# PACTHEMAN123/spMV-test

Hardware: AMD Instinct MI355X
Metric: fp32 CSR SpMV: achieved HBM GB/s (rocprofv3 FETCH_SIZE + WRITE_SIZE bytes of the K steps / wall time) (higher is better)
Workload: dtype f32; 1 GPU; c4: 16777216 x 16777216, nnz 268435456, row lengths 'mixed' mean 16, banded columns (band 8192), seed 20251031; variant=auto, rows_per_gpu=16777216, nnz_per_gpu=268435456, parallelism=single GPU, devices=1 ranks on 1 device(s), launch=one process, algorithmic_bytes_per_gpu=2348810244, hbm_bytes_per_gpu=1840380781

## Files before the change

include/spmv_hip.h:

```cpp
#ifndef SPMV_HIP_H
#define SPMV_HIP_H

#include <stdint.h>

#if defined(__GNUC__)
#define SPMV_API __attribute__((visibility("default")))
#else
#define SPMV_API
#endif

#ifdef __cplusplus
extern "C" {
#endif

typedef struct spmv_csr spmv_csr_t;

enum spmv_status {
    SPMV_OK = 0,
    SPMV_ERR_NO_DEVICE = -1,
    SPMV_ERR_INVALID = -2,
    SPMV_ERR_HIP = -3,
    SPMV_ERR_VARIANT = -4,
    SPMV_ERR_NOT_PLANNED = -5,
    SPMV_ERR_STALE_PLAN = -6
// ... 96 lines not shown
SPMV_API int spmv_csr_color(const spmv_csr_t *a, uint32_t seed, void *stream, int32_t *d_color ,
                            int32_t *d_perm , int32_t *color_ptr , int cap ,
                            int64_t info[8]);
SPMV_API int spmv_csr_permute(const spmv_csr_t *a, const int32_t *d_row_perm ,
                              const int32_t *d_col_perm , int flags, void *stream, spmv_csr_t **out);
SPMV_API int spmv_csr_permute_values(spmv_csr_t *b, const spmv_csr_t *a, void *stream);
SPMV_API int spmv_csr_permute_gather(const spmv_csr_t *b, int count, const void *d_src, int64_t src_stride, void *d_dst,
                                     int64_t dst_stride, void *stream);
SPMV_API int64_t spmv_csr_permute_map_bytes(const spmv_csr_t *b);
SPMV_API int spmv_permute_vector(const int32_t *d_perm, int64_t n, int inverse, const float *d_src, float *d_dst, void *stream);

SPMV_API int spmv_csr_plan(spmv_csr_t *h, int variant, void *stream);
SPMV_API int spmv_csr_run(spmv_csr_t *h, int variant, const float *d_x, float *d_y, void *stream);

SPMV_API int spmv_csr_values_changed(spmv_csr_t *h);

SPMV_API int spmv_csr_plan_get(const spmv_csr_t *h, int variant, int32_t params[8]);
SPMV_API int spmv_csr_plan_set(spmv_csr_t *h, int variant, const int32_t params[8], void *stream);
SPMV_API int spmv_csr_plan_like(spmv_csr_t *dst, const spmv_csr_t *src, int variant, void *stream);

SPMV_API int64_t spmv_csr_plan_bytes(const spmv_csr_t *h, int variant);

SPMV_API int spmv_csr_plan_describe(const spmv_csr_t *h, int variant, char *buf, int n);

SPMV_API int spmv_csr_time(spmv_csr_t *h, int variant, const float *d_x, float *d_y, int iters,
                  void *stream, float *ms_per_launch);

SPMV_API int spmv_csr_run_host(spmv_csr_t *h, int variant, const float *x_host, float *y_host,
                               float *kernel_ms);

SPMV_API int spmv_csr_spmm_plan(spmv_csr_t *h, void *stream);
SPMV_API int spmv_csr_spmm(spmv_csr_t *h, int k, const float *d_X, int64_t ldx, float *d_Y, int64_t ldy, void *stream);
SPMV_API int64_t spmv_csr_spmm_plan_bytes(const spmv_csr_t *h);
SPMV_API int spmv_csr_spmm_describe(const spmv_csr_t *h, char *buf, int n);

SPMV_API int spmv_csr_sddmm(spmv_csr_t *h, int k, const float *d_U, int64_t ldu, const float *d_X, int64_t ldx,
                            float *d_out, void *stream);

SPMV_API int spmv_csr_row_softmax(spmv_csr_t *h, float scale, const float *d_scores, float *d_out, void *stream);
SPMV_API int spmv_csr_row_softmax_backward(spmv_csr_t *h, float scale, const float *d_P, const float *d_dP,
                                           float *d_dS, void *stream);

SPMV_API int spmv_csr_attention_plan(spmv_csr_t *h, void *stream);
SPMV_API int64_t spmv_csr_attention_plan_bytes(const spmv_csr_t *h);
SPMV_API int spmv_csr_attention_forward(spmv_csr_t *h, float scale, int k, const float *d_Q, int64_t ldq, const float *d_K,
                                        int64_t ldk, int kv, const float *d_V, int64_t ldv, float *d_O, int64_t ldo,
// ... 162 lines not shown
```

spmv-test_amd/capi.py:

```python
from __future__ import annotations

import ctypes as C
import os
from pathlib import Path

PKG_DIR = Path(__file__).resolve().parent
LIB_PATH = PKG_DIR / "lib" / "libspmv_hip.so"
LAUNCHERS_PATH = PKG_DIR / "lib" / "libspmv_launchers.so"
TESTER_PATH = PKG_DIR / "bin" / "sparse_sgemv"
DIST_LIB_PATH = PKG_DIR / "lib" / "libspmv_dist.so"
DIST_SELFTEST_PATH = PKG_DIR / "bin" / "spmv_dist_selftest"

SCALAR, WAVE, WAVE_PIPE, VECTOR, ADAPTIVE, TILED, PANEL, AUTO, XSKIP = range(9)
VARIANTS = {"scalar": SCALAR, "wave": WAVE, "wave_pipe": WAVE_PIPE, "vector": VECTOR,
            "adaptive": ADAPTIVE, "tiled": TILED, "panel": PANEL, "auto": AUTO}
ALL_VARIANTS = dict(VARIANTS, xskip=XSKIP)

OK, ERR_NO_DEVICE, ERR_INVALID, ERR_HIP, ERR_VARIANT, ERR_NOT_PLANNED, ERR_STALE_PLAN = 0, -1, -2, -3, -4, -5, -6

_i32p, _f32p, _vp = C.c_void_p, C.c_void_p, C.c_void_p
_H = C.c_void_p
_HP = C.POINTER(C.c_void_p)


# ... 59 lines not shown
    "spmv_csr_spmm_plan": (C.c_int, [_H, _vp]),
    "spmv_csr_spmm": (C.c_int, [_H, C.c_int, _f32p, C.c_int64, _f32p, C.c_int64, _vp]),
    "spmv_csr_spmm_plan_bytes": (C.c_int64, [_H]),
    "spmv_csr_spmm_describe": (C.c_int, [_H, C.c_char_p, C.c_int]),
    "spmv_csr_sddmm": (C.c_int, [_H, C.c_int, _f32p, C.c_int64, _f32p, C.c_int64, _f32p, _vp]),
    "spmv_csr_spmm_16": (C.c_int, [_H, C.c_int, C.c_int, _vp, C.c_int64, _vp, C.c_int64, _vp]),
    "spmv_csr_sddmm_16": (C.c_int, [_H, C.c_int, C.c_int, _vp, C.c_int64, _vp, C.c_int64, _f32p, _vp]),
    "spmv_csr_spmm_plan_cols": (C.c_int, [_H, C.c_int, _vp]),
    "spmv_csr_spmm_cols": (C.c_int, [_H, C.c_int, C.c_int, _vp, C.c_int64, _vp, C.c_int64, _vp]),
    "spmv_csr_sddmm_cols": (C.c_int, [_H, C.c_int, C.c_int, _vp, C.c_int64, _vp, C.c_int64, _f32p, _vp]),
    "spmv_csr_row_softmax": (C.c_int, [_H, C.c_float, _f32p, _f32p, _vp]),
    "spmv_csr_row_softmax_backward": (C.c_int, [_H, C.c_float, _f32p, _f32p, _f32p, _vp]),
    "spmv_csr_attention_plan": (C.c_int, [_H, _vp]),
    "spmv_csr_attention_plan_bytes": (C.c_int64, [_H]),
    "spmv_csr_attention_plan_heads": (C.c_int, [_H, C.c_int, _vp]),
    "spmv_csr_attention_max_heads": (C.c_int, [_H, C.c_int, C.c_int]),
    "spmv_csr_attention_plan_wide": (C.c_int, [_H, C.c_int, _vp]),
    "spmv_csr_attention_max_heads_wide": (C.c_int, [_H, C.c_int, C.c_int]),
    "spmv_csr_plan_get": (C.c_int, [_H, C.c_int, C.POINTER(C.c_int32)]),
    "spmv_csr_plan_set": (C.c_int, [_H, C.c_int, C.POINTER(C.c_int32), _vp]),
    "spmv_csr_plan_like": (C.c_int, [_H, _H, C.c_int, _vp]),
    "spmv_csr_plan_bytes": (C.c_int64, [_H, C.c_int]),
    "spmv_csr_plan_describe": (C.c_int, [_H, C.c_int, C.c_char_p, C.c_int]),
    "spmv_csr_time": (C.c_int, [_H, C.c_int, _f32p, _f32p, C.c_int, _vp, C.POINTER(C.c_float)]),
    "spmv_csr_run_host": (C.c_int, [_H, C.c_int, _f32p, _f32p, C.POINTER(C.c_float)]),
    "spmv_dense_gemv": (C.c_int, [C.c_int, C.c_int, _f32p, _f32p, _f32p, C.c_int, _vp]),
    "spmv_dense_gemv_workspace_bytes": (C.c_int64, [C.c_int, C.c_int]),
    "spmv_dense_gemv_ws": (C.c_int, [C.c_int, C.c_int, _f32p, _f32p, _f32p, C.c_int, _vp, C.c_int64, _vp]),
    "spmv_asp_retile": (C.c_int, [C.c_int, C.c_int, _f32p, _f32p, _vp]),
    "spmv_asp_gemv_ws": (C.c_int, [C.c_int, C.c_int, _f32p, _f32p, _f32p, _vp, C.c_int64, _vp]),
    "spmv_dense_gemv_host": (C.c_int, [C.c_int, C.c_int, _f32p, _f32p, _f32p, C.c_int, C.POINTER(C.c_float)]),
    "spmv_tcsr_from_dense_host": (C.c_int, [C.c_int, C.c_int, _f32p, _vp, _HP]),
    "spmv_tcsr_from_dense_device": (C.c_int, [C.c_int, C.c_int, _f32p, _vp, _HP]),
    "spmv_tcsr_sizes": (C.c_int, [_H, C.POINTER(C.c_int64), C.POINTER(C.c_int64), C.POINTER(C.c_int64)]),
    "spmv_tcsr_download": (C.c_int, [_H, _i32p, _i32p, _f32p]),
    "spmv_tcsr_run": (C.c_int, [_H, _f32p, _f32p, _vp]),
    "spmv_tcsr_run_host": (C.c_int, [_H, _f32p, _f32p, C.POINTER(C.c_float)]),
    "spmv_tcsr_destroy": (C.c_int, [_H]),
    "spmv_bitmap_from_dense_host": (C.c_int, [C.c_int, C.c_int, C.c_int, _f32p, _vp, _HP]),
    "spmv_bitmap_from_dense_device": (C.c_int, [C.c_int, C.c_int, C.c_int, _f32p, _vp, _HP]),
    "spmv_bitmap_sizes": (C.c_int, [_H, C.POINTER(C.c_int64), C.POINTER(C.c_int64), C.POINTER(C.c_int32)]),
    "spmv_bitmap_download": (C.c_int, [_H, _i32p, _f32p]),
    "spmv_bitmap_run": (C.c_int, [_H, _f32p, _f32p, _vp]),
    "spmv_bitmap_run_host": (C.c_int, [_H, _f32p, _f32p, C.POINTER(C.c_float)]),
    "spmv_bitmap_destroy": (C.c_int, [_H]),
    "spmv_synth_fill": (C.c_int, [C.c_uint64, C.c_int64, C.c_int64, C.c_int64, C.c_int64, C.c_int64,
# ... 768 lines not shown
        check(lib().spmv_csr_run_host(self._h, variant, _ptr(x), _ptr(y), C.byref(ms)))
        return ms.value

    def plan_params(self, variant: int):
        a = (C.c_int32 * 8)()
        check(lib().spmv_csr_plan_get(self._h, variant, a))
        return list(a)

    def plan_set(self, variant: int, params, stream=None) -> None:
        a = (C.c_int32 * 8)(*params)
        check(lib().spmv_csr_plan_set(self._h, variant, a, _stream_handle(stream)))

    def plan_like(self, other: "CsrMatrix", variant: int, stream=None) -> None:
        check(lib().spmv_csr_plan_like(self._h, other._h, variant, _stream_handle(stream)))

    def plan_describe(self, variant: int) -> str:
        buf = C.create_string_buffer(256)
        check(lib().spmv_csr_plan_describe(self._h, variant, buf, 256))
        return buf.value.decode()

    def plan_bytes(self, variant: int) -> int:
        return lib().spmv_csr_plan_bytes(self._h, variant)

    def download(self):
        import numpy as np
        rp = np.empty(self.rows + 1, np.int32)
        ci = np.empty(self.nnz, np.int32)
        va = np.empty(self.nnz, np.float32)
        check(lib().spmv_csr_download(self._h, _ptr(rp), _ptr(ci), _ptr(va)))
        return rp, ci, va

    def close(self) -> None:
        if self._h:
            check(lib().spmv_csr_destroy(self._h))
            self._h = C.c_void_p()
            self._keep = ()

    def __del__(self):
        try:
            self.close()
        except Exception:
            pass


class TcsrMatrix:

# ... 176 lines not shown
```

spmv-test_amd/csrc/capi.hip:

```cpp
#include <cctype>
#include <cstdarg>
#include <cstdint>
#include <cstdlib>
#include <cstring>
#include <new>
#include "spmv_internal.hpp"

namespace spmv {

static thread_local char g_err[512] = "";
static thread_local float g_first_launch_ms = 0.0f;

void set_error(const char *fmt, ...)
{
    va_list ap;
    va_start(ap, fmt);
    vsnprintf(g_err, sizeof g_err, fmt, ap);
    va_end(ap);
}

int hip_fail(hipError_t e, const char *what, const char *file, int line)
{
    set_error("HIP error %s:%d: %s (%s)", file, line, hipGetErrorString(e), what);
    return SPMV_ERR_HIP;
// ... 1825 lines not shown
        default: set_error("spmv_csr_plan_set: unknown variant %d", target); return SPMV_ERR_VARIANT;
    }
    if (rc == SPMV_OK && variant == SPMV_AUTO) h->auto_variant = target;
    return rc;
}

int spmv_csr_plan_like(spmv_csr_t *dst, const spmv_csr_t *src, int variant, void *stream)
{
    int32_t params[8];
    int rc = spmv_csr_plan_get(src, variant, params);
    return rc ? rc : spmv_csr_plan_set(dst, variant, params, stream);
}

int64_t spmv_csr_plan_bytes(const spmv_csr_t *h, int variant)
{
    if (!h) return 0;
    const PanelPlan &panel = variant == SPMV_AUTO ? h->plan_auto_panel : h->plan_panel;
    if (variant == SPMV_AUTO) variant = h->auto_variant;
    switch (variant) {
        case SPMV_ADAPTIVE:
            return (int64_t)(h->plan_adaptive.nchunks + 1) * 4 + (int64_t)h->plan_adaptive.nchunks * 8;
        case SPMV_TILED:
            return (int64_t)(h->plan_tiled.nchunks + 1) * 4 + (int64_t)h->plan_tiled.nchunks * 16 +
                   ((h->plan_tiled.n16 || h->plan_tiled.nsorted) ? (int64_t)h->plan_tiled.nchunks * 4 : 0) +
                   (int64_t)h->plan_tiled.n16 * 2 * h->plan_tiled.block * kNnzPerThread +
                   (int64_t)h->plan_tiled.nsorted * 4 * h->plan_tiled.block * kNnzPerThread +
                   (int64_t)h->plan_tiled.nblk_chunks * 256 * 4;
        case SPMV_XSKIP:
            return (int64_t)h->plan_xskip.nseg * 8 + ((int64_t)h->plan_xskip.nblocks + 1) * 4 +
                   (h->plan_xskip.slabs > 1 ? (int64_t)h->plan_xskip.nblocks * h->plan_xskip.slabs * 1024 * 8 : 0);
        case SPMV_PANEL: return panel_plan_bytes(panel, h->nnz);
        case SPMV_WAVE:
            if (h->nnz > 32 * h->rows) return 0;
            return (int64_t)h->plan_wave.n_long * 8 + (int64_t)h->plan_wave.pieces * 16;
        case SPMV_SCALAR:
        case SPMV_WAVE_PIPE:
            return (int64_t)h->plan_wave.n_long * 8 + (int64_t)h->plan_wave.pieces * 16 + h->plan_wave.blocks * 8;
        default: return 0;
    }
}

int spmv_csr_plan_describe(const spmv_csr_t *h, int variant, char *buf, int n)
{
    if (!h || !buf || n <= 0) { set_error("spmv_csr_plan_describe: bad argument"); return SPMV_ERR_INVALID; }
    const PanelPlan *panel = &h->plan_panel;
    if (variant == SPMV_AUTO) {
        if (h->auto_variant < 0) { snprintf(buf, (size_t)n, "not planned"); return SPMV_OK; }
        const int w = snprintf(buf, (size_t)n, "auto -> %s: ", spmv_variant_name(h->auto_variant));
        if (w < 0 || w >= n) return SPMV_OK;
        if (h->auto_variant != SPMV_PANEL) return spmv_csr_plan_describe(h, h->auto_variant, buf + w, n - w);
        panel = &h->plan_auto_panel;
        variant = SPMV_PANEL;
        buf += w;
        n -= w;
    }
    const ChunkPlan *p = variant == SPMV_ADAPTIVE ? &h->plan_adaptive : (variant == SPMV_TILED ? &h->plan_tiled : nullptr);
    if (variant == SPMV_VECTOR) snprintf(buf, (size_t)n, "lanes_per_row=%d", h->vector_width);
    else if (variant == SPMV_WAVE && h->nnz > 32 * h->rows) snprintf(buf, (size_t)n, "no plan (a wavefront per row)");
    else if (variant == SPMV_WAVE_PIPE || variant == SPMV_SCALAR || variant == SPMV_WAVE) {
        if (!h->plan_wave.ready) snprintf(buf, (size_t)n, "not planned (the first run plans)");
        else snprintf(buf, (size_t)n, "long_rows=%d pieces=%d block_rows=%d blocks=%lld blocks_with_x_window=%lld col16=%d", h->plan_wave.n_long,
                      h->plan_wave.pieces, h->plan_wave.block_rows, (long long)h->plan_wave.blocks, (long long)h->plan_wave.win_blocks,
// ... 286 lines not shown
```

spmv-test_amd/csrc/kernels_adaptive.hip:

```cpp
#include "spmv_internal.hpp"
#include "tiled_chunks.hpp"
#include "lane_group.hpp"

namespace spmv {

__device__ __forceinline__ int pad_idx(int i) { return i + (i >> 5); }
template <int BLOCK>
__device__ __forceinline__ void zero_pad_words(float *smem, int tid)
{
    for (int h = tid; h < (chunk_of(BLOCK) >> 5); h += BLOCK) smem[h * 33 + 32] = 0.0f;
}

__device__ __forceinline__ int xcd_chunk(int bid, int n)
{
    const int q = n / kXcds, rem = n % kXcds;
    const int j = bid % kXcds, idx = bid / kXcds;
    return j * q + (j < rem ? j : rem) + idx;
}

struct Segment {
    int s, e;
    float *dst;
};

// ... 433 lines not shown
}

template <int BLOCK, bool TILED, bool PERSIST, typename E = float>
__global__ __launch_bounds__(BLOCK, waves_per_simd(BLOCK, PERSIST))
void k_adaptive(int64_t rows, int64_t nnz, int64_t cols, int chunk0, int nrun, const int32_t *__restrict__ row_ptr,
                const int32_t *__restrict__ col_idx, const E *__restrict__ vals, const float *__restrict__ x,
                float *__restrict__ y, const int32_t *__restrict__ chunk_lb, float *__restrict__ carry,
                const int32_t *__restrict__ win, const int32_t *__restrict__ list, int kRegion)
{
    extern __shared__ __attribute__((aligned(16))) float smem[];
    __shared__ ChunkShared<BLOCK> sh;
    adaptive_body<BLOCK, TILED, PERSIST, E>(smem, sh, (int)blockIdx.x, (int)gridDim.x, rows, nnz, cols, chunk0, nrun, row_ptr,
                                            col_idx, vals, x, y, chunk_lb, carry, win, list, kRegion);
}


__device__ __forceinline__ unsigned col16_at(const u4 (&raw)[2], int j, int q)
{
    const int e = (j & 1) * 4 + q;
    const unsigned word = raw[j >> 1][e >> 1];
    return (e & 1) ? (word >> 16) : (word & 0xffffu);
}

template <int BLOCK, bool BLOCKS, typename E = float>
__device__ __forceinline__ void tiled16_body(float *smem, ChunkShared<BLOCK> &sh, int bid, int64_t rows, int64_t cols,
                                             int nrun, const int32_t *__restrict__ row_ptr,
                                             const uint16_t *__restrict__ col16, const E *__restrict__ vals,
                                             const float *__restrict__ x, float *__restrict__ y,
                                             const int32_t *__restrict__ chunk_lb, float *__restrict__ carry,
                                             const int32_t *__restrict__ win, const int32_t *__restrict__ list,
                                             int kRegionArg, const int32_t *__restrict__ blk)
{
    constexpr int kVec = kNnzPerThread / 4;
    static_assert(kNnzPerThread == 16, "the col16 lane layout is two 16-byte loads of eight offsets");

    const int tid = threadIdx.x;
    const int ci = xcd_chunk(bid, nrun);
    const ChunkHead h = chunk_head<BLOCK>(sh, tid, list ? list[ci] : ci, chunk_lb);
    const int c = h.c;
    const int w0 = win[2 * c];
    const int wl = win[2 * c + 1];
    const int wlen = wl & kLenMask;
    const bool by_blocks = BLOCKS && (wl & kBlockBit);
    const int kRegion = by_blocks ? (kRegionArg / kBlkCols) * kBlkCols : kRegionArg;

    u4 raw[2];
    vals4_t<E> vv[kVec];
    {
        const u4 *c8 = reinterpret_cast<const u4 *>(col16 + h.base);
        const vals4_t<E> *v4 = value_vectors(vals, h.base);
        raw[0] = __builtin_nontemporal_load(&c8[tid]);
        raw[1] = __builtin_nontemporal_load(&c8[BLOCK + tid]);
#pragma unroll
        for (int j = 0; j < kVec; ++j) vv[j] = stream_load<BLOCK>(v4, tid, j);
    }
    const RowBounds b0 = first_bounds(tid, h, row_ptr);

    f4 xv[kVec];
#pragma unroll
    for (int j = 0; j < kVec; ++j)
#pragma unroll
        for (int q = 0; q < 4; ++q) xv[j][q] = 0.0f;
    if (wlen <= kRegion && wlen > 0) {
        if (by_blocks) stage_blocks<BLOCK>(x, blk + (int64_t)c * kBlkMax, wlen / kBlkCols, cols, smem, tid);
        else stage_slice<BLOCK, true>(x, (int64_t)w0, wlen, cols, smem, tid);
        __syncthreads();
#pragma unroll
        for (int j = 0; j < kVec; ++j)
#pragma unroll
            for (int q = 0; q < 4; ++q) xv[j][q] = smem[col16_at(raw, j, q)];
        __syncthreads();
    } else {
        for (int off = 0; off < wlen; off += kRegion) {
            const int len = (wlen - off) < kRegion ? (wlen - off) : kRegion;
            const int64_t g0 = (int64_t)w0 + off;
            if (by_blocks) stage_blocks<BLOCK>(x, blk + (int64_t)c * kBlkMax + off / kBlkCols, len / kBlkCols, cols, smem, tid);
            else stage_slice<BLOCK, true>(x, g0, len, cols, smem, tid);
            __syncthreads();
#pragma unroll
            for (int j = 0; j < kVec; ++j)
#pragma unroll
                for (int q = 0; q < 4; ++q) {
                    const unsigned o = col16_at(raw, j, q) - (unsigned)off;
                    if (o < (unsigned)len) xv[j][q] = smem[o];
                }
            __syncthreads();
        }
    }

    stage_products<BLOCK, E>(smem, tid, vv, [&](int j, int q, int) { return xv[j][q]; });
    __syncthreads();
    reduce_chunk<BLOCK, true, BLOCKS ? 1 : 0>(smem, sh, tid, h.c, h.lb0, h.m, h.base, h.lim, row_ptr, y, carry, b0.rb, b0.re);
}

template <int BLOCK, bool BLOCKS, typename E = float>
__global__ __launch_bounds__(BLOCK, 8)
void k_tiled16(int64_t rows, int64_t cols, int nrun, const int32_t *__restrict__ row_ptr, const uint16_t *__restrict__ col16,
               const E *__restrict__ vals, const float *__restrict__ x, float *__restrict__ y,
               const int32_t *__restrict__ chunk_lb, float *__restrict__ carry, const int32_t *__restrict__ win,
               const int32_t *__restrict__ list, int kRegion, const int32_t *__restrict__ blk)
{
    extern __shared__ __attribute__((aligned(16))) float smem[];
    __shared__ ChunkShared<BLOCK> sh;
    tiled16_body<BLOCK, BLOCKS, E>(smem, sh, (int)blockIdx.x, rows, cols, nrun, row_ptr, col16, vals, x, y, chunk_lb, carry, win,
                                   list, kRegion, blk);
}

template <int BLOCK, typename E = float>
__device__ __forceinline__ void sorted_body(float *smem, ChunkShared<BLOCK> &sh, int bid, int64_t rows, int nrun,
                                            const int32_t *__restrict__ row_ptr, const uint32_t *__restrict__ perm,
                                            const E *__restrict__ vals, const float *__restrict__ x,
                                            float *__restrict__ y, const int32_t *__restrict__ chunk_lb,
                                            float *__restrict__ carry, const int32_t *__restrict__ win,
                                            const int32_t *__restrict__ list)
{
    constexpr int kChunkT = chunk_of(BLOCK);
    constexpr int kVec = kNnzPerThread / 4;
    constexpr int kColBits = sorted_col_bits(BLOCK);
    constexpr unsigned kColMask = (1u << kColBits) - 1u;

    const int tid = threadIdx.x;
    const int ci = xcd_chunk(bid, nrun);
    const ChunkHead h = chunk_head<BLOCK>(sh, tid, list[ci], chunk_lb);
    const float *xw = x + win[2 * h.c];

    u4 pw[kVec];
    vals4_t<E> vv[kVec];
    {
        const u4 *p4 = reinterpret_cast<const u4 *>(perm + (int64_t)ci * kChunkT);
        const vals4_t<E> *v4 = value_vectors(vals, h.base);
#pragma unroll
        for (int j = 0; j < kVec; ++j) pw[j] = stream_load<BLOCK>(p4, tid, j);
#pragma unroll
        for (int j = 0; j < kVec; ++j) vv[j] = stream_load<BLOCK>(v4, tid, j);
    }
    const RowBounds b0 = first_bounds(tid, h, row_ptr);

#pragma unroll
    for (int j = 0; j < kVec; ++j) {
        float g[4];
#pragma unroll
        for (int q = 0; q < 4; ++q) g[q] = xw[pw[j][q] & kColMask];
#pragma unroll
        for (int q = 0; q < 4; ++q) smem[pad_idx((int)(pw[j][q] >> kColBits))] = g[q];
    }
    __syncthreads();
    stage_products<BLOCK, E>(smem, tid, vv, [&](int, int, int w) { return smem[w]; });
    __syncthreads();
    reduce_chunk<BLOCK, true>(smem, sh, tid, h.c, h.lb0, h.m, h.base, h.lim, row_ptr, y, carry, b0.rb, b0.re);
}

template <int BLOCK, typename E = float>
__global__ __launch_bounds__(BLOCK, 8)
void k_sorted(int64_t rows, int nrun, const int32_t *__restrict__ row_ptr, const uint32_t *__restrict__ perm,
              const E *__restrict__ vals, const float *__restrict__ x, float *__restrict__ y,
              const int32_t *__restrict__ chunk_lb, float *__restrict__ carry, const int32_t *__restrict__ win,
              const int32_t *__restrict__ list)
{
    extern __shared__ __attribute__((aligned(16))) float smem[];
    __shared__ ChunkShared<BLOCK> sh;
    sorted_body<BLOCK, E>(smem, sh, (int)blockIdx.x, rows, nrun, row_ptr, perm, vals, x, y, chunk_lb, carry, win, list);
}

template <int BLOCK, bool BLOCKS, typename E = float>
__global__ __launch_bounds__(BLOCK, 8)
void k_tiled_mixed(int64_t rows, int64_t nnz, int64_t cols, int n32, int nsorted, int n16, const int32_t *__restrict__ row_ptr,
                   const int32_t *__restrict__ col_idx, const uint16_t *__restrict__ col16, const uint32_t *__restrict__ perm,
                   const E *__restrict__ vals, const float *__restrict__ x, float *__restrict__ y,
                   const int32_t *__restrict__ chunk_lb, float *__restrict__ carry, const int32_t *__restrict__ win,
                   const int32_t *__restrict__ list32, const int32_t *__restrict__ list_sorted,
                   const int32_t *__restrict__ list16, int kRegion, const int32_t *__restrict__ blk)
{
    extern __shared__ __attribute__((aligned(16))) float smem[];
    __shared__ ChunkShared<BLOCK> sh;
    const int b = (int)blockIdx.x;
    if (b < n32)
        adaptive_body<BLOCK, true, false, E>(smem, sh, b, n32, rows, nnz, cols, 0, n32, row_ptr, col_idx, vals, x,
                                             y, chunk_lb, carry, win, list32, kRegion);
    else if (b < n32 + nsorted)
        sorted_body<BLOCK, E>(smem, sh, b - n32, rows, nsorted, row_ptr, perm, vals, x, y, chunk_lb, carry, win, list_sorted);
    else
        tiled16_body<BLOCK, BLOCKS, E>(smem, sh, b - n32 - nsorted, rows, cols, n16, row_ptr, col16, vals, x, y, chunk_lb,
                                       carry, win, list16, kRegion, blk);
}

__global__ void k_carry_fixup(int nchunks, int chunk, const int32_t *__restrict__ row_ptr,
                              const int32_t *__restrict__ chunk_lb, const float *__restrict__ carry,
                              float *__restrict__ y)
{
    int c = blockIdx.x * blockDim.x + threadIdx.x;
    if (c >= nchunks - 1) return;
    const int lb0 = chunk_lb[c], lb1 = chunk_lb[c + 1];
    if (lb1 == lb0) return;
    const int64_t r = (int64_t)lb1 - 1;
    const int64_t endp = row_ptr[r + 1];
    if (endp <= (int64_t)(c + 1) * chunk) return;
    float s = y[r];
    for (int64_t c2 = c + 1; c2 * chunk < endp; ++c2) s += carry[c2];
    y[r] = s;
}

__global__ __launch_bounds__(256)
void k_plan_windows(int64_t nnz, int64_t cols, int nchunks, int chunk, const int32_t *__restrict__ col_idx,
                    int32_t *__restrict__ win, int32_t *__restrict__ stats, int region, int maxpass, int sorted_from,
                    int sorted_span, PlanCost cost, const int32_t *__restrict__ lb, const int32_t *__restrict__ row_ptr)
{
// ... 145 lines not shown
    int grid = nrun;
    if (PERSIST) {
        const int res = resident_workgroups(h.device, BLOCK, waves_per_simd(BLOCK, true));
        if (grid > res) grid = res;
    }
    return launch_region<k_adaptive<BLOCK, TILED, PERSIST, E>>("k_adaptive", h, p, grid, BLOCK, s, h.rows, h.nnz, h.cols, chunk0, nrun,
                                                               h.d_row_ptr, h.d_col_idx, vals, x, y, p.d_lb, p.d_carry, p.d_win,
                                                               (const int32_t *)nullptr, p.region);
}

template <int BLOCK, bool BLOCKS, typename E>
static int launch_tiled16(const spmv_csr &h, const ChunkPlan &p, const E *vals, const float *x, float *y, hipStream_t s)
{
    if (p.n16 <= 0) return SPMV_OK;
    return launch_region<k_tiled16<BLOCK, BLOCKS, E>>("k_tiled16", h, p, p.n16, BLOCK, s, h.rows, h.cols, p.n16, h.d_row_ptr, p.d_col16,
                                                      vals, x, y, p.d_lb, p.d_carry, p.d_win,
                                                      p.n16 == p.nchunks ? (const int32_t *)nullptr : p.d_list16.get(), p.region, p.d_blk);
}

template <int BLOCK, bool BLOCKS, typename E>
static int launch_mixed(const spmv_csr &h, const ChunkPlan &p, const E *vals, const float *x, float *y, hipStream_t s)
{
    const int n32 = p.nchunks - p.n16 - p.nsorted;
    return launch_region<k_tiled_mixed<BLOCK, BLOCKS, E>>("k_tiled_mixed", h, p, p.nchunks, BLOCK, s, h.rows, h.nnz, h.cols, n32, p.nsorted,
                                                          p.n16, h.d_row_ptr, h.d_col_idx, p.d_col16, p.d_perm, vals, x, y, p.d_lb,
                                                          p.d_carry, p.d_win, p.d_list32, p.d_list_sorted, p.d_list16, p.region, p.d_blk);
}

template <int BLOCK, typename E>
static int launch_sorted(const spmv_csr &h, const ChunkPlan &p, const E *vals, const float *x, float *y, hipStream_t s)
{
    return launch_region<k_sorted<BLOCK, E>>("k_sorted", h, p, p.nsorted, BLOCK, s, h.rows, p.nsorted, h.d_row_ptr, p.d_perm, vals, x,
                                             y, p.d_lb, p.d_carry, p.d_win, p.d_list_sorted);
}

template <int BLOCK, bool TILED, typename E>
static int launch_either(bool persist, const spmv_csr &h, const ChunkPlan &p, const E *vals, const float *x, float *y, hipStream_t s)
{
    if constexpr (TILED) {
        if (!persist && (p.n16 > 0 || p.nsorted > 0)) {
            const bool lists = p.nblk_chunks > 0;
            if (p.n16 == p.nchunks)
                return lists ? launch_tiled16<BLOCK, true>(h, p, vals, x, y, s) : launch_tiled16<BLOCK, false>(h, p, vals, x, y, s);
            if (p.nsorted == p.nchunks) return launch_sorted<BLOCK>(h, p, vals, x, y, s);
            return lists ? launch_mixed<BLOCK, true>(h, p, vals, x, y, s) : launch_mixed<BLOCK, false>(h, p, vals, x, y, s);
        }
    }
    if constexpr (kIs16<E>) {
        return launch_range<BLOCK, TILED, false>(h, p, vals, 0, p.nchunks, x, y, s);
// ... 49 lines not shown
```

spmv-test_amd/csrc/plan_adaptive.hip:

```cpp
#include <climits>
#include <cstdlib>
#include <cstring>
#include "spmv_internal.hpp"
#include "tiled_chunks.hpp"

namespace spmv {

__global__ void k_plan_chunks(int64_t rows, int nchunks, int chunk, const int32_t *__restrict__ row_ptr,
                              int32_t *__restrict__ lb)
{
    int c = blockIdx.x * blockDim.x + threadIdx.x;
    if (c > nchunks) return;
    if (c == nchunks) { lb[c] = (int32_t)rows; return; }
    const int64_t key = (int64_t)c * chunk;
    int64_t lo = 0, hi = rows;
    while (lo < hi) {
        int64_t mid = (lo + hi) >> 1;
        if ((int64_t)row_ptr[mid] < key) lo = mid + 1; else hi = mid;
    }
    lb[c] = (int32_t)lo;
}

template <int BLOCK>
__global__ __launch_bounds__(BLOCK) void k_plan_sorted(const int32_t *__restrict__ col_idx,
// ... 335 lines not shown
        p.nblk_chunks = 0;
        (void)p.d_col16.reset();
        (void)p.d_blk.reset();
    }
    return SPMV_OK;
}

static int count_block_list_chunks(const spmv_csr &h, ChunkPlan &p, hipStream_t s, int *out)
{
    *out = 0;
    if (p.nchunks == 0 || !p.d_win) return SPMV_OK;
    DevPtr<int32_t> nblk, some;
    SPMV_HIP_TRY(nblk.alloc(1));
    SPMV_HIP_TRY(some.alloc(1));
    SPMV_HIP_TRY(hipMemsetAsync(nblk.get(), 0, sizeof(int32_t), s));
    if (int rc = run_plan_col16(h, p, nullptr, nblk.get(), some.get(), 1, s)) return rc;
    int32_t cnt = 0;
    SPMV_HIP_TRY(hipMemcpyAsync(&cnt, nblk.get(), sizeof cnt, hipMemcpyDeviceToHost, s));
    SPMV_HIP_TRY(hipStreamSynchronize(s));
    *out = cnt;
    return SPMV_OK;
}

static int build_lists(const spmv_csr &h, ChunkPlan &p, hipStream_t s)
{
    (void)p.d_list16.reset();
    (void)p.d_list32.reset();
    (void)p.d_list_sorted.reset();
    (void)p.d_perm.reset();
    p.n16 = p.nsorted = 0;
    if (p.nchunks == 0 || !p.d_win || p.persist) return SPMV_OK;
    int rc;
    DevPtr<int32_t> f16, fs, t16, ts;
    SPMV_HIP_TRY(f16.alloc((size_t)p.nchunks));
    SPMV_HIP_TRY(fs.alloc((size_t)p.nchunks));
    SPMV_HIP_TRY(t16.alloc(1));
    SPMV_HIP_TRY(ts.alloc(1));
    const unsigned g = (unsigned)((p.nchunks + 255) / 256);
    hipLaunchKernelGGL(k_plan_kinds, dim3(g), dim3(256), 0, s, p.nchunks, p.d_win, f16.get(), fs.get());
    if ((rc = check_launch("k_plan_kinds"))) return rc;
    if ((rc = exclusive_scan_i32(f16.get(), p.nchunks, t16.get(), s))) return rc;
    if ((rc = exclusive_scan_i32(fs.get(), p.nchunks, ts.get(), s))) return rc;
    int32_t n16 = 0, ns = 0;
    SPMV_HIP_TRY(hipMemcpyAsync(&n16, t16.get(), sizeof(int32_t), hipMemcpyDeviceToHost, s));
    SPMV_HIP_TRY(hipMemcpyAsync(&ns, ts.get(), sizeof(int32_t), hipMemcpyDeviceToHost, s));
    SPMV_HIP_TRY(hipStreamSynchronize(s));
    p.n16 = n16;
    p.nsorted = ns;
    if (n16 == 0 && ns == 0) return SPMV_OK;
    SPMV_HIP_TRY(p.d_list16.alloc((size_t)n16));
    SPMV_HIP_TRY(p.d_list_sorted.alloc((size_t)ns));
    SPMV_HIP_TRY(p.d_list32.alloc((size_t)(p.nchunks - n16 - ns)));
    hipLaunchKernelGGL(k_plan_lists, dim3(g), dim3(256), 0, s, p.nchunks, p.d_win, f16.get(), fs.get(), p.d_list16, p.d_list_sorted,
                       p.d_list32);
    if ((rc = check_launch("k_plan_lists"))) return rc;
    if (ns > 0) {
        SPMV_HIP_TRY(p.d_perm.alloc((size_t)chunk_of(p.block) * (size_t)ns));
        rc = dispatch_block(p.block, [&](auto B) {
            constexpr int BLOCK = decltype(B)::value;
            hipLaunchKernelGGL((k_plan_sorted<BLOCK>), dim3(p.nchunks), dim3(BLOCK), 0, s, h.d_col_idx, p.d_win, fs.get(), p.d_perm);
            return check_launch("k_plan_sorted");
        });
        if (rc) return rc;
    }
    SPMV_HIP_TRY(hipStreamSynchronize(s));
    return SPMV_OK;
}

static int finish_tiled(spmv_csr &h, bool col16, hipStream_t s)
{
    int rc = col16 ? build_col16(h, h.plan_tiled, s) : SPMV_OK;
    if (rc == SPMV_OK) rc = build_lists(h, h.plan_tiled, s);
    if (rc) h.plan_tiled = ChunkPlan{};
    return rc;
}

int plan_tiled_with(spmv_csr &h, int block, int maxpass, bool col16, hipStream_t s)
{
    if ((block != 256 && block != 512 && block != 1024) || maxpass < 1 || maxpass > 64) {
        set_error("tiled plan: block %d / maxpass %d outside 256|512|1024 / 1..64", block, maxpass);
        return SPMV_ERR_INVALID;
    }
    const int rc = build_plan(h, block, maxpass, s, h.plan_tiled, nullptr, nullptr);
    return rc ? rc : finish_tiled(h, col16, s);
}

int plan_adaptive_with(spmv_csr &h, int block, hipStream_t s)
{
// ... 146 lines not shown
```

spmv-test_amd/csrc/spmv_internal.hpp:

```cpp
#pragma once
#include <hip/hip_runtime.h>
#include <atomic>
#include <cstdint>
#include <cstdio>
#include <utility>
#include "spmv_hip.h"
#include "attention_args.hpp"

namespace spmv {

void set_error(const char *fmt, ...) __attribute__((format(printf, 1, 2)));
int hip_fail(hipError_t e, const char *what, const char *file, int line);

#define SPMV_HIP_TRY(call)                                                   \
    do {                                                                     \
        hipError_t e__ = (call);                                             \
        if (e__ != hipSuccess) return ::spmv::hip_fail(e__, #call, __FILE__, __LINE__); \
    } while (0)

static inline int check_launch(const char *what)
{
    hipError_t e = hipGetLastError();
    if (e != hipSuccess) return hip_fail(e, what, __FILE__, __LINE__);
    return SPMV_OK;
// ... 46 lines not shown
constexpr int kMaxHeads = 65535;

#ifndef SPMV_T_NPT
#define SPMV_T_NPT 16
#endif
#ifndef SPMV_T_SHORT
#define SPMV_T_SHORT 32
#endif
constexpr int kNnzPerThread = SPMV_T_NPT;
constexpr int kShortSeg = SPMV_T_SHORT;

struct ChunkPlan {
    int block = 0;
    int nchunks = 0;
    DevPtr<int32_t> d_lb;
    DevPtr<float> d_carry;
    DevPtr<int32_t> d_win;
    DevPtr<uint16_t> d_col16;
    DevPtr<int32_t> d_list16;
    DevPtr<int32_t> d_list32;
    int n16 = 0;
    DevPtr<uint32_t> d_perm;
    DevPtr<int32_t> d_list_sorted;
    int nsorted = 0;
    int nsorted_marked = 0;
    int sorted_from = 0;
    int long_piece_chunks = 0;
    double model_cost = 0.0;
    DevPtr<int32_t> d_blk;
    int nblk_chunks = 0;
    int maxpass = 0;
    bool col16_wanted = false;
    int spanning_rows = 0;
    int region = 0;
    bool persist = false;
    int staged_single = 0;
    int staged_full = 0;
};

struct ValuesStamp {
    uint64_t gen = 0;
    uint64_t sum = 0;
    bool have_sum = false;
};

enum class PanelLayout { none = 0, sweep_l2 = 1, sweep_lds = 2, sorted_blocks = 3, binned = 4, binned_scattered = 5 };
// ... 435 lines not shown
```

spmv-test_amd/csrc/tiled_chunks.hpp:

```cpp
#pragma once
#include <type_traits>
#include "spmv_internal.hpp"

namespace spmv {

using i4 = int __attribute__((ext_vector_type(4)));
using f4 = float __attribute__((ext_vector_type(4)));
using u4 = unsigned __attribute__((ext_vector_type(4)));

#ifndef SPMV_T_GROUP
#define SPMV_T_GROUP 16
#endif
constexpr int kGroup = SPMV_T_GROUP;

__host__ __device__ constexpr int chunk_of(int block) { return block * kNnzPerThread; }
__host__ __device__ constexpr int prod_words(int block) { return chunk_of(block) + (chunk_of(block) >> 5); }
__host__ __device__ constexpr int region_words(int block) { return (block / 256) * 4832; }
static_assert(region_words(256) >= prod_words(256), "region must hold the products");
__host__ __device__ constexpr int max_long(int block) { return chunk_of(block) / (kShortSeg + 1) + 2; }
#ifndef SPMV_T_HUGE
#define SPMV_T_HUGE 512
#endif
constexpr int kHugeSeg = SPMV_T_HUGE;
__host__ __device__ constexpr int max_huge(int block) { return chunk_of(block) / (kHugeSeg + 1) + 2; }

template <typename F>
int dispatch_block(int block, F &&f)
{
    if (block == 256) return f(std::integral_constant<int, 256>{});
    if (block == 512) return f(std::integral_constant<int, 512>{});
    return f(std::integral_constant<int, 1024>{});
}

constexpr int kOutsideBit = 1 << 30;
constexpr int kCol16Bit = 1 << 29;
constexpr int kBlockBit = 1 << 28;
constexpr int kSortedBit = 1 << 27;
constexpr int kLenMask = kSortedBit - 1;
#ifndef SPMV_T_SORTED_FROM
#define SPMV_T_SORTED_FROM (-1)
#endif
constexpr int kSortedFromDefault = SPMV_T_SORTED_FROM;
__host__ __device__ constexpr int sorted_pos_bits(int block) { return block == 1024 ? 14 : (block == 512 ? 13 : 12); }
__host__ __device__ constexpr int sorted_col_bits(int) { return 18; }
static_assert(sorted_pos_bits(1024) + sorted_col_bits(1024) <= 32, "one word per nonzero");
#ifndef SPMV_T_BLKBITS
#define SPMV_T_BLKBITS 8
#endif
constexpr int kBlkBits = SPMV_T_BLKBITS;
constexpr int kBlkCols = 1 << kBlkBits;
constexpr int kBlkMax = 65536 / kBlkCols;

struct PlanCost {
    int c16_base = 788, c16_pass = 110, c32_base = 1075, c32_pass = 123, sorted_base = 1075, sorted_line_512 = 1792,
        sorted_line_1024 = 1485, sorted_few_rows = 205, unstaged = 3072, long_piece = 512;
};

int launch_plan_windows(const spmv_csr &h, const ChunkPlan &p, int32_t *d_stats, const PlanCost &cost, hipStream_t s);

}
```

Baseline: 5479 GB/s.

## Run mixed tiled chunks in identity order instead of per-format lists

When most chunks use the col16 format, the mixed tiled kernel maps each block straight to its chunk in natural order and branches on the window flags, instead of reading list16/list_sorted/list32 indirection arrays. Value vectors are loaded before dispatch so the stream load can be issued early. The last partial chunk is swapped so it is not scheduled last. The intent is to keep neighbouring chunks' x windows adjacent in time, which should improve reuse of x in L2, and to drop the list lookups. The cost is a divergent branch per block and a mix of chunk formats within each wave of blocks. An optional window-first staging switch is added but is off by default.

```diff
diff --git a/include/spmv_hip.h b/include/spmv_hip.h
--- a/include/spmv_hip.h
+++ b/include/spmv_hip.h
@@ -142,6 +142,8 @@
 SPMV_API int64_t spmv_csr_plan_bytes(const spmv_csr_t *h, int variant);
 
 SPMV_API int spmv_csr_plan_describe(const spmv_csr_t *h, int variant, char *buf, int n);
+
+SPMV_API int spmv_csr_plan_chunk_order(const spmv_csr_t *h, int variant);
 
 SPMV_API int spmv_csr_time(spmv_csr_t *h, int variant, const float *d_x, float *d_y, int iters,
                   void *stream, float *ms_per_launch);
diff --git a/spmv-test_amd/capi.py b/spmv-test_amd/capi.py
--- a/spmv-test_amd/capi.py
+++ b/spmv-test_amd/capi.py
@@ -105,6 +105,7 @@
     "spmv_csr_plan_like": (C.c_int, [_H, _H, C.c_int, _vp]),
     "spmv_csr_plan_bytes": (C.c_int64, [_H, C.c_int]),
     "spmv_csr_plan_describe": (C.c_int, [_H, C.c_int, C.c_char_p, C.c_int]),
+    "spmv_csr_plan_chunk_order": (C.c_int, [_H, C.c_int]),
     "spmv_csr_time": (C.c_int, [_H, C.c_int, _f32p, _f32p, C.c_int, _vp, C.POINTER(C.c_float)]),
     "spmv_csr_run_host": (C.c_int, [_H, C.c_int, _f32p, _f32p, C.POINTER(C.c_float)]),
     "spmv_dense_gemv": (C.c_int, [C.c_int, C.c_int, _f32p, _f32p, _f32p, C.c_int, _vp]),
@@ -919,6 +920,12 @@
     def plan_bytes(self, variant: int) -> int:
         return lib().spmv_csr_plan_bytes(self._h, variant)
 
+    def plan_chunk_order(self, variant: int) -> int:
+        rc = lib().spmv_csr_plan_chunk_order(self._h, variant)
+        if rc < 0:
+            check(rc)
+        return rc
+
     def download(self):
         import numpy as np
         rp = np.empty(self.rows + 1, np.int32)
diff --git a/spmv-test_amd/csrc/capi.hip b/spmv-test_amd/csrc/capi.hip
--- a/spmv-test_amd/csrc/capi.hip
+++ b/spmv-test_amd/csrc/capi.hip
@@ -1871,7 +1871,8 @@
             return (int64_t)(h->plan_adaptive.nchunks + 1) * 4 + (int64_t)h->plan_adaptive.nchunks * 8;
         case SPMV_TILED:
             return (int64_t)(h->plan_tiled.nchunks + 1) * 4 + (int64_t)h->plan_tiled.nchunks * 16 +
-                   ((h->plan_tiled.n16 || h->plan_tiled.nsorted) ? (int64_t)h->plan_tiled.nchunks * 4 : 0) +
+                   ((h->plan_tiled.identity_order ? h->plan_tiled.nsorted : (h->plan_tiled.n16 || h->plan_tiled.nsorted))
+                        ? (int64_t)h->plan_tiled.nchunks * 4 : 0) +
                    (int64_t)h->plan_tiled.n16 * 2 * h->plan_tiled.block * kNnzPerThread +
                    (int64_t)h->plan_tiled.nsorted * 4 * h->plan_tiled.block * kNnzPerThread +
                    (int64_t)h->plan_tiled.nblk_chunks * 256 * 4;
@@ -1887,6 +1888,17 @@
             return (int64_t)h->plan_wave.n_long * 8 + (int64_t)h->plan_wave.pieces * 16 + h->plan_wave.blocks * 8;
         default: return 0;
     }
+}
+
+int spmv_csr_plan_chunk_order(const spmv_csr_t *h, int variant)
+{
+    if (!h) { set_error("spmv_csr_plan_chunk_order: null handle"); return SPMV_ERR_INVALID; }
+    if (variant == SPMV_AUTO) variant = h->auto_variant;
+    if (variant != SPMV_TILED) { set_error("spmv_csr_plan_chunk_order: SPMV_TILED, or SPMV_AUTO resolved to it"); return SPMV_ERR_VARIANT; }
+    const ChunkPlan &p = h->plan_tiled;
+    if (!p.block) { set_error("SPMV_TILED used before spmv_csr_plan"); return SPMV_ERR_NOT_PLANNED; }
+    const bool mixed = !p.persist && (p.n16 > 0 || p.nsorted > 0) && p.n16 != p.nchunks && p.nsorted != p.nchunks;
+    return !mixed ? 0 : (p.identity_order ? 2 : 1);
 }
 
 int spmv_csr_plan_describe(const spmv_csr_t *h, int variant, char *buf, int n)
diff --git a/spmv-test_amd/csrc/kernels_adaptive.hip b/spmv-test_amd/csrc/kernels_adaptive.hip
--- a/spmv-test_amd/csrc/kernels_adaptive.hip
+++ b/spmv-test_amd/csrc/kernels_adaptive.hip
@@ -479,21 +479,26 @@
     return (e & 1) ? (word >> 16) : (word & 0xffffu);
 }
 
-template <int BLOCK, bool BLOCKS, typename E = float>
-__device__ __forceinline__ void tiled16_body(float *smem, ChunkShared<BLOCK> &sh, int bid, int64_t rows, int64_t cols,
-                                             int nrun, const int32_t *__restrict__ row_ptr,
+__device__ __forceinline__ int listed_chunk(int bid, int nrun, const int32_t *__restrict__ list)
+{
+    const int ci = xcd_chunk(bid, nrun);
+    return list ? list[ci] : ci;
+}
+
+template <int BLOCK, bool BLOCKS, typename E = float, bool PRE = false>
+__device__ __forceinline__ void tiled16_body(float *smem, ChunkShared<BLOCK> &sh, int c0, int64_t rows, int64_t cols,
+                                             const int32_t *__restrict__ row_ptr,
                                              const uint16_t *__restrict__ col16, const E *__restrict__ vals,
                                              const float *__restrict__ x, float *__restrict__ y,
                                              const int32_t *__restrict__ chunk_lb, float *__restrict__ carry,
-                                             const int32_t *__restrict__ win, const int32_t *__restrict__ list,
-                                             int kRegionArg, const int32_t *__restrict__ blk)
+                                             const int32_t *__restrict__ win, int kRegionArg,
+                                             const int32_t *__restrict__ blk, const vals4_t<E> *pre = nullptr)
 {
     constexpr int kVec = kNnzPerThread / 4;
     static_assert(kNnzPerThread == 16, "the col16 lane layout is two 16-byte loads of eight offsets");
 
     const int tid = threadIdx.x;
-    const int ci = xcd_chunk(bid, nrun);
-    const ChunkHead h = chunk_head<BLOCK>(sh, tid, list ? list[ci] : ci, chunk_lb);
+    const ChunkHead h = chunk_head<BLOCK>(sh, tid, c0, chunk_lb);
     const int c = h.c;
     const int w0 = win[2 * c];
     const int wl = win[2 * c + 1];
@@ -509,18 +514,27 @@
         raw[0] = __builtin_nontemporal_load(&c8[tid]);
         raw[1] = __builtin_nontemporal_load(&c8[BLOCK + tid]);
 #pragma unroll
-        for (int j = 0; j < kVec; ++j) vv[j] = stream_load<BLOCK>(v4, tid, j);
-    }
-    const RowBounds b0 = first_bounds(tid, h, row_ptr);
-
-    f4 xv[kVec];
-#pragma unroll
-    for (int j = 0; j < kVec; ++j)
-#pragma unroll
-        for (int q = 0; q < 4; ++q) xv[j][q] = 0.0f;
-    if (wlen <= kRegion && wlen > 0) {
+        for (int j = 0; j < kVec; ++j) {
+            if constexpr (PRE) vv[j] = pre[j];
+            else vv[j] = stream_load<BLOCK>(v4, tid, j);
+        }
+    }
+    const bool one_pass = wlen <= kRegion && wlen > 0;
+    auto stage_window = [&] {
         if (by_blocks) stage_blocks<BLOCK>(x, blk + (int64_t)c * kBlkMax, wlen / kBlkCols, cols, smem, tid);
         else stage_slice<BLOCK, true>(x, (int64_t)w0, wlen, cols, smem, tid);
+    };
+    constexpr bool kFirst = kWindowFirst && !BLOCKS;
+    if (kFirst && one_pass) stage_window();
+    const RowBounds b0 = first_bounds(tid, h, row_ptr);
+
+    f4 xv[kVec];
+#pragma unroll
+    for (int j = 0; j < kVec; ++j)
+#pragma unroll
+        for (int q = 0; q < 4; ++q) xv[j][q] = 0.0f;
+    if (one_pass) {
+        if (!kFirst) stage_window();
         __syncthreads();
 #pragma unroll
         for (int j = 0; j < kVec; ++j)
@@ -559,17 +573,17 @@
 {
     extern __shared__ __attribute__((aligned(16))) float smem[];
     __shared__ ChunkShared<BLOCK> sh;
-    tiled16_body<BLOCK, BLOCKS, E>(smem, sh, (int)blockIdx.x, rows, cols, nrun, row_ptr, col16, vals, x, y, chunk_lb, carry, win,
-                                   list, kRegion, blk);
-}
-
-template <int BLOCK, typename E = float>
-__device__ __forceinline__ void sorted_body(float *smem, ChunkShared<BLOCK> &sh, int bid, int64_t rows, int nrun,
+    tiled16_body<BLOCK, BLOCKS, E>(smem, sh, listed_chunk((int)blockIdx.x, nrun, list), rows, cols, row_ptr, col16, vals, x, y,
+                                   chunk_lb, carry, win, kRegion, blk);
+}
+
+template <int BLOCK, typename E = float, bool PRE = false>
+__device__ __forceinline__ void sorted_body(float *smem, ChunkShared<BLOCK> &sh, int c0, int ci, int64_t rows,
                                             const int32_t *__restrict__ row_ptr, const uint32_t *__restrict__ perm,
                                             const E *__restrict__ vals, const float *__restrict__ x,
                                             float *__restrict__ y, const int32_t *__restrict__ chunk_lb,
                                             float *__restrict__ carry, const int32_t *__restrict__ win,
-                                            const int32_t *__restrict__ list)
+                                            const vals4_t<E> *pre = nullptr)
 {
     constexpr int kChunkT = chunk_of(BLOCK);
     constexpr int kVec = kNnzPerThread / 4;
@@ -577,8 +591,7 @@
     constexpr unsigned kColMask = (1u << kColBits) - 1u;
 
     const int tid = threadIdx.x;
-    const int ci = xcd_chunk(bid, nrun);
-    const ChunkHead h = chunk_head<BLOCK>(sh, tid, list[ci], chunk_lb);
+    const ChunkHead h = chunk_head<BLOCK>(sh, tid, c0, chunk_lb);
     const float *xw = x + win[2 * h.c];
 
     u4 pw[kVec];
@@ -589,7 +602,10 @@
 #pragma unroll
         for (int j = 0; j < kVec; ++j) pw[j] = stream_load<BLOCK>(p4, tid, j);
 #pragma unroll
-        for (int j = 0; j < kVec; ++j) vv[j] = stream_load<BLOCK>(v4, tid, j);
+        for (int j = 0; j < kVec; ++j) {
+            if constexpr (PRE) vv[j] = pre[j];
+            else vv[j] = stream_load<BLOCK>(v4, tid, j);
+        }
     }
     const RowBounds b0 = first_bounds(tid, h, row_ptr);
 
@@ -616,7 +632,8 @@
 {
     extern __shared__ __attribute__((aligned(16))) float smem[];
     __shared__ ChunkShared<BLOCK> sh;
-    sorted_body<BLOCK, E>(smem, sh, (int)blockIdx.x, rows, nrun, row_ptr, perm, vals, x, y, chunk_lb, carry, win, list);
+    const int ci = xcd_chunk((int)blockIdx.x, nrun);
+    sorted_body<BLOCK, E>(smem, sh, list[ci], ci, rows, row_ptr, perm, vals, x, y, chunk_lb, carry, win);
 }
 
 template <int BLOCK, bool BLOCKS, typename E = float>
@@ -631,14 +648,48 @@
     extern __shared__ __attribute__((aligned(16))) float smem[];
     __shared__ ChunkShared<BLOCK> sh;
     const int b = (int)blockIdx.x;
+    if (kIdentityOrder && !BLOCKS && list16 == nullptr) {
+        const int32_t *__restrict__ sorted_slot = list_sorted;
+        constexpr int kChunkT = chunk_of(BLOCK);
+        constexpr int kVec = kNnzPerThread / 4;
+        const int nchunks = n32 + nsorted + n16;
+        int c = xcd_chunk(b, nchunks);
+        bool full = true;
+        if ((int64_t)nchunks * kChunkT != nnz) {
+            const int last = nchunks - 1, q = nchunks / kXcds;
+            const int first = q > 0 ? nchunks - q : last;
+            c = c == first ? last : (c == last ? first : c);
+            full = c != last;
+        }
+        if (full) {
+            vals4_t<E> vv[kVec];
+            const vals4_t<E> *v4 = value_vectors(vals, (int64_t)c * kChunkT);
+#pragma unroll
+            for (int j = 0; j < kVec; ++j) vv[j] = stream_load<BLOCK>(v4, (int)threadIdx.x, j);
+            const int wl = win[2 * c + 1];
+            if (wl & kCol16Bit) {
+                tiled16_body<BLOCK, BLOCKS, E, true>(smem, sh, c, rows, cols, row_ptr, col16, vals, x, y, chunk_lb, carry, win,
+                                                     kRegion, blk, vv);
+                return;
+            }
+            if (wl & kSortedBit) {
+                sorted_body<BLOCK, E, true>(smem, sh, c, sorted_slot[c], rows, row_ptr, perm, vals, x, y, chunk_lb, carry, win, vv);
+                return;
+            }
+        }
+        adaptive_body<BLOCK, true, false, E>(smem, sh, 0, 1, rows, nnz, cols, c, 1, row_ptr, col_idx, vals, x, y, chunk_lb,
+                                             carry, win, nullptr, kRegion);
+        return;
+    }
     if (b < n32)
         adaptive_body<BLOCK, true, false, E>(smem, sh, b, n32, rows, nnz, cols, 0, n32, row_ptr, col_idx, vals, x,
                                              y, chunk_lb, carry, win, list32, kRegion);
-    else if (b < n32 + nsorted)
-        sorted_body<BLOCK, E>(smem, sh, b - n32, rows, nsorted, row_ptr, perm, vals, x, y, chunk_lb, carry, win, list_sorted);
-    else
-        tiled16_body<BLOCK, BLOCKS, E>(smem, sh, b - n32 - nsorted, rows, cols, n16, row_ptr, col16, vals, x, y, chunk_lb,
-                                       carry, win, list16, kRegion, blk);
+    else if (b < n32 + nsorted) {
+        const int ci = xcd_chunk(b - n32, nsorted);
+        sorted_body<BLOCK, E>(smem, sh, list_sorted[ci], ci, rows, row_ptr, perm, vals, x, y, chunk_lb, carry, win);
+    } else
+        tiled16_body<BLOCK, BLOCKS, E>(smem, sh, listed_chunk(b - n32 - nsorted, n16, list16), rows, cols, row_ptr, col16, vals,
+                                       x, y, chunk_lb, carry, win, kRegion, blk);
 }
 
 __global__ void k_carry_fixup(int nchunks, int chunk, const int32_t *__restrict__ row_ptr,
@@ -830,9 +881,11 @@
 static int launch_mixed(const spmv_csr &h, const ChunkPlan &p, const E *vals, const float *x, float *y, hipStream_t s)
 {
     const int n32 = p.nchunks - p.n16 - p.nsorted;
+    const int32_t *list_sorted = p.identity_order ? p.d_sorted_slot.get() : p.d_list_sorted.get();
+    const int32_t *list16 = p.identity_order ? nullptr : p.d_list16.get();
     return launch_region<k_tiled_mixed<BLOCK, BLOCKS, E>>("k_tiled_mixed", h, p, p.nchunks, BLOCK, s, h.rows, h.nnz, h.cols, n32, p.nsorted,
                                                           p.n16, h.d_row_ptr, h.d_col_idx, p.d_col16, p.d_perm, vals, x, y, p.d_lb,
-                                                          p.d_carry, p.d_win, p.d_list32, p.d_list_sorted, p.d_list16, p.region, p.d_blk);
+                                                          p.d_carry, p.d_win, p.d_list32, list_sorted, list16, p.region, p.d_blk);
 }
 
 template <int BLOCK, typename E>
diff --git a/spmv-test_amd/csrc/plan_adaptive.hip b/spmv-test_amd/csrc/plan_adaptive.hip
--- a/spmv-test_amd/csrc/plan_adaptive.hip
+++ b/spmv-test_amd/csrc/plan_adaptive.hip
@@ -381,12 +381,24 @@
     return SPMV_OK;
 }
 
+static bool want_identity_order(int nchunks, int n16)
+{
+    if (!kIdentityOrder) return false;
+    if (const char *e = getenv("SPMV_TILED_ORDER")) {
+        if (!strcmp(e, "identity")) return true;
+        if (!strcmp(e, "lists")) return false;
+    }
+    return kIdentityShare > 0 && (int64_t)(nchunks - n16) * kIdentityShare <= nchunks;
+}
+
 static int build_lists(const spmv_csr &h, ChunkPlan &p, hipStream_t s)
 {
     (void)p.d_list16.reset();
     (void)p.d_list32.reset();
     (void)p.d_list_sorted.reset();
     (void)p.d_perm.reset();
+    (void)p.d_sorted_slot.reset();
+    p.identity_order = false;
     p.n16 = p.nsorted = 0;
     if (p.nchunks == 0 || !p.d_win || p.persist) return SPMV_OK;
     int rc;
@@ -407,12 +419,16 @@
     p.n16 = n16;
     p.nsorted = ns;
     if (n16 == 0 && ns == 0) return SPMV_OK;
-    SPMV_HIP_TRY(p.d_list16.alloc((size_t)n16));
-    SPMV_HIP_TRY(p.d_list_sorted.alloc((size_t)ns));
-    SPMV_HIP_TRY(p.d_list32.alloc((size_t)(p.nchunks - n16 - ns)));
-    hipLaunchKernelGGL(k_plan_lists, dim3(g), dim3(256), 0, s, p.nchunks, p.d_win, f16.get(), fs.get(), p.d_list16, p.d_list_sorted,
-                       p.d_list32);
-    if ((rc = check_launch("k_plan_lists"))) return rc;
+    const bool mixed = n16 != p.nchunks && ns != p.nchunks;
+    p.identity_order = mixed && p.nblk_chunks == 0 && want_identity_order(p.nchunks, n16);
+    if (!p.identity_order) {
+        SPMV_HIP_TRY(p.d_list16.alloc((size_t)n16));
+        SPMV_HIP_TRY(p.d_list_sorted.alloc((size_t)ns));
+        SPMV_HIP_TRY(p.d_list32.alloc((size_t)(p.nchunks - n16 - ns)));
+        hipLaunchKernelGGL(k_plan_lists, dim3(g), dim3(256), 0, s, p.nchunks, p.d_win, f16.get(), fs.get(), p.d_list16,
+                           p.d_list_sorted, p.d_list32);
+        if ((rc = check_launch("k_plan_lists"))) return rc;
+    }
     if (ns > 0) {
         SPMV_HIP_TRY(p.d_perm.alloc((size_t)chunk_of(p.block) * (size_t)ns));
         rc = dispatch_block(p.block, [&](auto B) {
@@ -423,6 +439,7 @@
         if (rc) return rc;
     }
     SPMV_HIP_TRY(hipStreamSynchronize(s));
+    if (p.identity_order && ns > 0) p.d_sorted_slot = std::move(fs);
     return SPMV_OK;
 }
 
diff --git a/spmv-test_amd/csrc/spmv_internal.hpp b/spmv-test_amd/csrc/spmv_internal.hpp
--- a/spmv-test_amd/csrc/spmv_internal.hpp
+++ b/spmv-test_amd/csrc/spmv_internal.hpp
@@ -92,6 +92,8 @@
     int n16 = 0;
     DevPtr<uint32_t> d_perm;
     DevPtr<int32_t> d_list_sorted;
+    DevPtr<int32_t> d_sorted_slot;
+    bool identity_order = false;
     int nsorted = 0;
     int nsorted_marked = 0;
     int sorted_from = 0;
diff --git a/spmv-test_amd/csrc/tiled_chunks.hpp b/spmv-test_amd/csrc/tiled_chunks.hpp
--- a/spmv-test_amd/csrc/tiled_chunks.hpp
+++ b/spmv-test_amd/csrc/tiled_chunks.hpp
@@ -44,6 +44,18 @@
 __host__ __device__ constexpr int sorted_pos_bits(int block) { return block == 1024 ? 14 : (block == 512 ? 13 : 12); }
 __host__ __device__ constexpr int sorted_col_bits(int) { return 18; }
 static_assert(sorted_pos_bits(1024) + sorted_col_bits(1024) <= 32, "one word per nonzero");
+#ifndef SPMV_T_IDENTITY_SHARE
+#define SPMV_T_IDENTITY_SHARE 8
+#endif
+constexpr int kIdentityShare = SPMV_T_IDENTITY_SHARE;
+#ifndef SPMV_T_IDENTITY_ORDER
+#define SPMV_T_IDENTITY_ORDER 1
+#endif
+constexpr bool kIdentityOrder = SPMV_T_IDENTITY_ORDER != 0;
+#ifndef SPMV_T_WINDOW_FIRST
+#define SPMV_T_WINDOW_FIRST 0
+#endif
+constexpr bool kWindowFirst = SPMV_T_WINDOW_FIRST != 0;
 #ifndef SPMV_T_BLKBITS
 #define SPMV_T_BLKBITS 8
 #endif
```

Result: faster. 5630 GB/s (median of 6 runs) (+2.8%).
